# zheminzhou/PEPPAN

Hardware: AMD Instinct MI355X
Metric: gene_pairs_aligned_per_s (higher is better)
Workload: dtype int16; 1 GPU; synthgenes-v1 seed 355: 10000 genes x 1002 nt, all-vs-all (BASELINE configs[2] search stage), min_id 0.45 min_ratio...; queries_per_rank=10000, reference_genes_per_rank=10000

## Files before the change

peppan_amd/csrc/capi.hip:

```cpp
#include "common.h"
#include "setstate.h"
#include <chrono>
#include <time.h>
#include <algorithm>
#include <cmath>
#include <cstring>
#include <new>

int pep_fail(pep_ctx *ctx, int code, const std::string &msg)
{
    if (ctx) { ctx->n_down = 0; ctx->pin_down_used = 0; }
    if (ctx) {
        ctx->err = msg;
        ctx->n_pending = 0;
        ctx->pin_small_used = 0;
        for (LookbackState &st : ctx->lookback) st.dirty = true;
        ctx->zero_clean = false;
        for (bool &f : ctx->zero_ok) f = false;
        ctx->set_clean_slots = 0;
    }
    return code;
}

int dev_reserve(pep_ctx *ctx, DevBuf &b, size_t bytes)
// ... 459 lines not shown
int32_t pep_min_score_ka(uint32_t qlen, double dbsize, double max_evalue, double ka_lambda, double ka_k)
{
    const double s = log(ka_k * (double)qlen * dbsize / max_evalue) / ka_lambda;
    const int32_t r = (int32_t)ceil(s);
    return r < 1 ? 1 : r;
}

int32_t pep_min_score(uint32_t qlen, double dbsize, double max_evalue)
{
    return pep_min_score_ka(qlen, dbsize, max_evalue, 0.267, 0.041);
}

int pep_ctx_create(int device, pep_ctx **out)
{
    if (!out) return PEP_ERR_ARG;
    *out = nullptr;
    int n = 0;
    if (hipGetDeviceCount(&n) != hipSuccess || device < 0 || device >= n) return PEP_ERR_HIP;
    pep_ctx *ctx = new (std::nothrow) pep_ctx();
    if (!ctx) return PEP_ERR_INTERNAL;
    ctx->device = device;
    memset(&ctx->stats, 0, sizeof(ctx->stats));
    pep_default_params(&ctx->params);
    if (hipSetDevice(device) != hipSuccess) { delete ctx; return PEP_ERR_HIP; }
    if (hipStreamCreate(&ctx->stream.s) != hipSuccess) { delete ctx; return PEP_ERR_HIP; }
    if (pin_reserve(ctx, ctx->pin_small, 16384) != PEP_OK) { *out = ctx; return PEP_ERR_HIP; }
    int rc = pep_selftest_dpp(ctx);
    if (rc != PEP_OK) { *out = ctx; return rc; }
    *out = ctx;
    return PEP_OK;
}

pep_ctx::~pep_ctx()
{
    (void)hipSetDevice(device);
    pep_drop_dev_result(this);
    pep_materialise_staged(this);
}

void pep_ctx_destroy(pep_ctx *ctx) { delete ctx; }

int pep_live_resources(uint64_t *device_bytes, uint64_t *pinned_bytes, uint32_t *events)
{
    if (!device_bytes || !pinned_bytes || !events) return PEP_ERR_ARG;
    *device_bytes = pep_live.device_bytes; *pinned_bytes = pep_live.pinned_bytes; *events = pep_live.events;
    return PEP_OK;
// ... 456 lines not shown
```

peppan_amd/csrc/common.h:

```cpp
#pragma once
#include <hip/hip_runtime.h>
#include <stdint.h>
#include <stddef.h>
#include <atomic>
#include <optional>
#include <string>
#include <type_traits>
#include <vector>
#include "../../include/peppan_hip.h"
using CallTimes = struct pep_call_times;

#define PEP_WAVE 64
#define PEP_TAB_REP 16

#define PEP_HIP(ctx, expr)                                                                            \
    do {                                                                                              \
        hipError_t _e = (expr);                                                                       \
        if (_e != hipSuccess) {                                                                       \
            return pep_fail((ctx), PEP_ERR_HIP, std::string(#expr) + ": " + hipGetErrorString(_e));   \
        }                                                                                             \
    } while (0)

#define PEP_TRY(expr)                  \
    do {                               \
        int _rc = (expr);              \
        if (_rc != PEP_OK) return _rc; \
// ... 121 lines not shown
    PEP_WS_TRACE_DIRS = PEP_WS_IDX_PART,
    PEP_WS_SW_SCAN_IN = 14,
    PEP_WS_SW_ORDER = 15,
    PEP_WS_SEL = 19,
    PEP_WS_SEL_RUNS_KEYS = 20,
    PEP_WS_RUNS = 21,
    PEP_WS_KEEP = 22,
    PEP_WS_HITS_OUT = 23,
    PEP_WS_COUNT
};

enum PepLookback {
    PEP_LB_SCAN_U32 = 0,
    PEP_LB_SCAN_U64,
    PEP_LB_SELECT_COUNT,
    PEP_LB_SELECT_RUNS,
    PEP_LB_TOPK_HITS,
    PEP_LB_TOPK_RUNS,
    PEP_LB_SORT,
    PEP_LB_COUNT
};

struct LookbackState { DevBuf buf; uint32_t epoch = 0, ticket_base = 0; bool dirty = false; };

enum PepTimer { TM_SEED = 0, TM_TOTAL, TM_SW, TM_SW_TRACE, TM_TRACE, TM_MATCH0, TM_MATCH1, TM_MATCH2, TM_MATCH3, TM_COUNT };

struct pep_ctx {
    int device = 0;
    Stream stream;
    PinBuf pin_small;
    size_t pin_small_used = 0;
    struct PendingRead { void *dst; size_t off, n; } pending[32];
    int n_pending = 0;
    PinBuf pin_k1, pin_k1q;
    DevBuf d_k1_desc_q, d_k1_desc_t;
    DevBuf d_self_delta, d_self_t;
    const uint32_t *self_first = nullptr;
    uint32_t self_first_cnt = 0;
    int self_exact_len = 0;
    Event k1_event;
    Event k1q_event;
    Event wait_event;
    Event k1_t0, k1_t1;
    PinBuf pin_up;
    size_t pin_up_used = 0;
    Event up_event;
// ... 30 lines not shown
        std::vector<pep_target_meta> t_meta;
        DevBuf d_off, d_len, d_desc;
        DevBuf d_first;
        uint32_t n_first = 0;
    } nucl_q, nucl_t;
    int nucl_strands = 0;
    DevBuf d_min_score;
    DevBuf d_trace_defer;
    DevBuf d_trace_mode;
    std::vector<uint32_t> group_of_seq;
    DevBuf d_t_class;
    DevBuf d_t_subject;
    DevBuf ws[PEP_WS_COUNT];
    DevBuf sub_lds;
    DevBuf d_params;
    int8_t d_params_host[1024] = {};
    bool d_params_valid = false;
    Event tm_a[TM_COUNT], tm_b[TM_COUNT];
    int tm_state[TM_COUNT] = {};
    int timing_level = 0;
    PinBuf pin_labels;
    uint64_t trace_swept = 0;
    LookbackState lookback[PEP_LB_COUNT];
    DevBuf sort_hist;
    DevBuf d_set;
    uint64_t set_clean_slots = 0;
    DevBuf uf_nodes;
    std::vector<uint32_t> uf_nodes_host;
    struct { bool pending = false; pep_result *res = nullptr; const void *d_hits = nullptr, *d_cig = nullptr; const uint32_t *d_n_hits = nullptr; uint64_t n_bound = 0; bool grouped = false; } ext;
    struct { void *d_dst = nullptr; const void *pinned_src = nullptr; uint64_t n_words = 0; } upload;
    bool want_nt_match = false;
    DevBuf d_nt_match;
    PinBuf pin_nt_match;
    uint32_t grp_nodes = 0, grp_q_base = 0;
    bool device_results = false;
    pep_result *dev_result = nullptr;
    DevBuf d_zero;
    bool zero_clean = false;
    DevBuf d_mail_copy;
    bool zero_ok[4] = {false, false, false, false};
    CallTimes calls[PEP_CALL_COUNT] = {};
    uint64_t k16_serial = 0;
    DevBuf k16_tri, k16_leader;
    DevBuf k17[11];
    uint64_t k18_n_conf = 0, k18_n_walk = 0;
    DevBuf k18[18];
// ... 102 lines not shown
int pep_read_back_with_upload(pep_ctx *ctx, void *dst, const void *d_src, size_t n, void *d_up_dst, const void *pinned_up_src, uint64_t n_up_words);
struct pep_key_unpack { int on, tb, bb; uint32_t bin_min; };
int pep_sort_u64(pep_ctx *ctx, uint64_t *d_keys, uint64_t *d_tmp, const uint32_t *d_n, uint64_t n_bound, int bits, uint32_t *d_hist_zeroed,
                 const pep_key_unpack *unpack);
int pep_sort_u64_two_level(pep_ctx *ctx, uint64_t *d_keys, uint64_t *d_tmp, uint64_t n, int bits, const uint32_t *d_top_hist, const pep_key_unpack *unpack);
int pep_k1_query_queue(pep_ctx *ctx, int gtable), pep_k1_query_take(pep_ctx *ctx);
int pep_k1_ref_queue(pep_ctx *ctx, int frames, int gtable), pep_k1_ref_take(pep_ctx *ctx);
int pep_k1_host_tables(pep_ctx *ctx, PepSide side);
int pep_nucl_sets(pep_ctx *ctx, int strands);
int pep_find_candidates(pep_ctx *ctx, uint64_t **d_cands, uint64_t *n_cands, int (*before_sync)(pep_ctx *) = nullptr, int (*need_targets)(pep_ctx *) = nullptr);
int pep_upload_sub_table(pep_ctx *ctx);
int pep_sw_run(pep_ctx *ctx, const uint64_t *d_cands, uint64_t n, bool trace, const int32_t *d_known = nullptr, const int32_t *d_end_lane = nullptr, const int32_t *d_skip_mode = nullptr,
               const uint32_t *d_n = nullptr, uint64_t dir_blocks_bound = 0, unsigned long long **d_hdr = nullptr);
int pep_extend(pep_ctx *ctx, const uint64_t *d_cands, uint64_t n_cands, const int32_t *h_min_score, pep_result *res, bool defer = false, bool group = false);
int pep_extend_finish(pep_ctx *ctx);
int pep_selftest_dpp(pep_ctx *ctx);
int pep_k7_hits_queue(pep_ctx *ctx, uint64_t n_hits, const pep_hit *d_hits, const uint32_t *d_cigar, const uint32_t *d_n_hits = nullptr);
int pep_k10_queue(pep_ctx *ctx, uint64_t n_hits, const pep_hit *d_hits, const uint32_t *d_n_hits = nullptr);
int pep_k10_components_dev(pep_ctx *ctx, uint32_t n_nodes, uint64_t n_hits, const pep_hit *d_hits, uint32_t q_base, const uint32_t *h_node_of_target,
                           uint64_t n_targets, uint32_t *h_label);

static inline uint64_t ceil_div(uint64_t a, uint64_t b) { return (a + b - 1) / b; }

__device__ __forceinline__ unsigned long long pep_band_cells(int Lq, int Lt, int dlo)
{
    const int dl = max(dlo, -(Lq - 1)), dh = min(dlo + 127, Lt - 1);
    if (dl > dh) return 0ull;
    auto tri = [](long long a, long long b) { return b < a ? 0ll : (a + b) * (b - a + 1) / 2; };
    const long long k = (long long)Lt - Lq;
    const long long flat_hi = min((long long)dh, k), slope_lo = max((long long)dl, k + 1);
    long long total = (flat_hi >= dl ? (flat_hi - dl + 1) * (long long)Lq : 0ll);
    if (slope_lo <= dh) total += (long long)(dh - slope_lo + 1) * Lt - tri(slope_lo, dh);
    total += tri(dl, min((long long)dh, -1ll));
    return (unsigned long long)total;
}

__device__ __forceinline__ uint32_t uf_root(uint32_t *parent, uint32_t x)
{
    for (;;) {
        const uint32_t p = __hip_atomic_load(&parent[x], __ATOMIC_RELAXED, __HIP_MEMORY_SCOPE_AGENT);
        if (p == x) return x;
        x = p;
    }
}
__device__ __forceinline__ void uf_unite(uint32_t *parent, uint32_t x, uint32_t y)
{
// ... 15 lines not shown
```

peppan_amd/csrc/sw.hip:

```cpp
#include "common.h"
#include "lookback.h"

namespace {

constexpr int LDS_TABLE_BYTES = 256 * PEP_TAB_REP * 4;
constexpr int TAB_ROW_SHIFT = PEP_TAB_REP == 32 ? 7 : 6;
constexpr int WAVES_PER_BLOCK = 8;

constexpr int LEN_BUCKETS = 1024;
__device__ __forceinline__ uint32_t len_bucket(uint32_t nb) { return nb < (uint32_t)LEN_BUCKETS ? nb : (uint32_t)LEN_BUCKETS - 1; }

struct SwArgs {
    const uint64_t *cands;
    uint64_t n;
    const uint8_t *q_res, *t_res;
    const uint32_t *q_off, *q_len, *t_off, *t_len;
    const uint32_t *sub_image;
    const uint64_t *dir_off;
    const uint32_t *nblk;
    uint32_t *dirs;
    int4 *out;
    int oe, ext;
    int lds_res_bytes;
    uint32_t *defer;
// ... 578 lines not shown
}

__global__ __launch_bounds__(64 * WAVES_PER_BLOCK, 4) void sw_trace_retry_kernel(SwArgs a)
{
    extern __shared__ __attribute__((aligned(16))) unsigned char smem[];
    const unsigned long long n_list = a.counts[6];
    if ((unsigned long long)blockIdx.x * WAVES_PER_BLOCK >= n_list) return;
    uint32_t *lds_tab = reinterpret_cast<uint32_t *>(smem);
    for (int x = threadIdx.x; x < LDS_TABLE_BYTES / 4; x += blockDim.x) lds_tab[x] = a.sub_image[x];
    __syncthreads();
    const int lane = threadIdx.x & 63, wave = threadIdx.x >> 6;
    uint16_t *lds_res = reinterpret_cast<uint16_t *>(smem + LDS_TABLE_BYTES + (size_t)wave * a.lds_res_bytes);
    const SwArgs *ka = (const SwArgs *)__builtin_amdgcn_kernarg_segment_ptr();
    for (;;) {
        unsigned long long w = 0;
        if (lane == 0) w = atomicAdd(a.counts + 7, 1ull);
        w = ((unsigned long long)(unsigned int)__builtin_amdgcn_readfirstlane((int)(w >> 32)) << 32) | (unsigned int)__builtin_amdgcn_readfirstlane((int)w);
        if (w >= n_list) break;
        trace_slow_path(ka, (uint64_t)a.defer[w], smem, lds_res, lane, 1);
    }
}

struct IdentArgs { int8_t diag[32]; uint32_t dominant, harmless; };
__global__ __launch_bounds__(256) void identical_check(const uint64_t *__restrict__ cands, uint64_t n, const uint8_t *__restrict__ q_res, const uint32_t *__restrict__ q_off,
                                                       const uint32_t *__restrict__ q_len, const uint8_t *__restrict__ t_res, const uint32_t *__restrict__ t_off,
                                                       const uint32_t *__restrict__ t_len, IdentArgs ia, int4 *__restrict__ out, int32_t *__restrict__ settled)
{
    const int lane = threadIdx.x & 63;
    const uint64_t c = (uint64_t)blockIdx.x * 4 + (threadIdx.x >> 6);
    if (c >= n) return;
    const uint64_t key = cands[c];
    const uint32_t q = (uint32_t)(key >> 43), t = (uint32_t)((key >> 18) & ((1u << 25) - 1));
    const int bin = (int)(key & ((1u << 18) - 1));
    const int dlo = bin * 64 - (1 << 23) - 32;
    const int L = (int)q_len[q];
    const int my_diag = ia.diag[lane & 31];
    bool same = L > 0 && L == (int)t_len[t] && dlo <= 0 && dlo + 127 >= 0;
    bool tail = false;
    int sum = 0;
    if (same) {
        const uint8_t *qg = q_res + q_off[q], *tg = t_res + t_off[t];
        for (int x0 = 0; x0 < L && same; x0 += 256) {
            uint32_t qa[4], ta[4];
#pragma unroll
            for (int k = 0; k < 4; ++k) { const int x = x0 + 64 * k + lane; qa[k] = x < L ? qg[x] : 0u; ta[k] = x < L ? tg[x] : 0u; }
#pragma unroll
            for (int k = 0; k < 4; ++k) {
                const bool in = x0 + 64 * k + lane < L;
                const int d = __shfl(my_diag, (int)(qa[k] & 31u), 64);
                const bool dom = in && qa[k] < 32u && ((ia.dominant >> qa[k]) & 1u), harm = in && qa[k] < 32u && ((ia.harmless >> qa[k]) & 1u);
                const unsigned long long m_dom = __ballot(dom), m_harm = __ballot(harm);
                const bool bad = __ballot(in && (qa[k] != ta[k] || !(dom || harm))) != 0ull
                                 || (m_dom && (tail || (m_harm && (63 - __builtin_clzll(m_dom)) > (__builtin_ffsll((long long)m_harm) - 1))));
                if (bad) same = false;
                if (dom) sum += d;
                tail = tail || m_harm != 0ull;
            }
        }
    }
#pragma unroll
    for (int d = 32; d > 0; d >>= 1) sum += __shfl_xor(sum, d, 64);
    same = same && sum > 0;
    if (lane == 0) {
        settled[c] = same ? -2 : 0;
        if (same) out[c] = make_int4(sum, (-dlo) >> 1, -1, (-dlo) >> 1);
    }
}

__global__ __launch_bounds__(256) void sw_prep(const uint64_t *__restrict__ cands, uint64_t n_host, const uint32_t *__restrict__ d_n, const uint32_t *__restrict__ q_len,
                                               const uint32_t *__restrict__ t_len, uint32_t *__restrict__ nblk, uint64_t *__restrict__ nblk64,
                                               unsigned long long *__restrict__ cells_total,
                                               uint32_t *__restrict__ len_hist,
                                               uint32_t nb_limit,
                                               const int32_t *__restrict__ skip_mode,
                                               int count_skipped,
                                               uint64_t *__restrict__ dir_off,
                                               LbLaunch lb)
{
    __shared__ uint32_t lh[LEN_BUCKETS];
    __shared__ uint32_t s_tile;
    for (int x = threadIdx.x; x < LEN_BUCKETS; x += 256) lh[x] = 0;
    __syncthreads();
    const uint64_t n = d_n ? (uint64_t)*d_n : n_host;
    const uint32_t tile = lb.state ? lb_take_tile(lb.state, lb.ticket_base, &s_tile) : blockIdx.x;
    const uint64_t c = (uint64_t)tile * 256 + threadIdx.x;
    unsigned long long cells = 0, blocks = 0, cells_skipped = 0, n_skipped = 0;
    bool is_long = false;
    const bool skipped = c < n && skip_mode && skip_mode[c] == -2;
// ... 139 lines not shown
    PEP_TRY(pep_zero_block(ctx, trace ? PEP_ZC_SW_TRACE : PEP_ZC_SW_SCORE, trace ? PEP_ZERO_SW_TRACE : PEP_ZERO_SW_SCORE, PEP_ZERO_SW_BYTES, &zb));
    PEP_TRY(dev_reserve(ctx, ctx->ws[PEP_WS_SW_ORDER], (n + 1) * sizeof(uint32_t)));
    unsigned long long *cells = reinterpret_cast<unsigned long long *>(zb);
    if (d_hdr) *d_hdr = cells;
    uint32_t *len_hist = reinterpret_cast<uint32_t *>(reinterpret_cast<unsigned char *>(zb) + 64), *cursor = len_hist + LEN_BUCKETS, *order = ctx->ws[PEP_WS_SW_ORDER].as<uint32_t>();
    LbLaunch lb = {nullptr, 0, 0};
    const uint64_t prep_tiles = ceil_div(n + (trace ? 1 : 0), 256);
    if (trace) PEP_TRY(pep_lookback_begin(ctx, PEP_LB_SCAN_U64, prep_tiles, 1, 48, &lb));
    const int32_t *skip = trace ? d_skip_mode : nullptr;
    if (!trace && (P.reserved2 & 2) == 0 && (n >= 16384 || (P.reserved2 & 4)) && P.gap_ext >= 0 && P.gap_open + P.gap_ext > 0) {
        PEP_TRY(dev_reserve(ctx, ctx->ws[PEP_WS_SW_SKIP_MODE], (n + 1) * sizeof(int32_t)));
        IdentArgs ia;
        ia.dominant = ia.harmless = 0;
        for (int r = 0; r < 32; ++r) {
            ia.diag[r] = P.sub[r * 32 + r];
            bool dom = P.sub[r * 32 + r] > 0, harm = true;
            for (int x = 0; x < 32; ++x) {
                if (x != r) dom = dom && P.sub[r * 32 + x] < P.sub[r * 32 + r];
                harm = harm && P.sub[r * 32 + x] <= 0;
            }
            if (dom) ia.dominant |= 1u << r;
            if (harm) ia.harmless |= 1u << r;
        }
        hipLaunchKernelGGL(identical_check, dim3((unsigned)ceil_div(n, 4)), dim3(256), 0, ctx->stream, d_cands, n, ctx->q.res.as<const uint8_t>(), ctx->q.off.as<const uint32_t>(),
                           ctx->q.len.as<const uint32_t>(), ctx->t.res.as<const uint8_t>(), ctx->t.off.as<const uint32_t>(), ctx->t.len.as<const uint32_t>(), ia,
                           ctx->ws[PEP_WS_SW_OUT].as<int4>(), ctx->ws[PEP_WS_SW_SKIP_MODE].as<int32_t>());
        skip = ctx->ws[PEP_WS_SW_SKIP_MODE].as<const int32_t>();
    }
    hipLaunchKernelGGL(sw_prep, dim3((unsigned)prep_tiles), dim3(256), 0, ctx->stream, d_cands, n, trace ? d_n : nullptr, ctx->q.len.as<const uint32_t>(),
                       ctx->t.len.as<const uint32_t>(), ctx->ws[PEP_WS_SW_NBLK].as<uint32_t>(), ctx->ws[PEP_WS_SW_SCAN_IN].as<uint64_t>(), cells, len_hist, nb_limit, skip, trace ? 0 : 1,
                       ctx->ws[PEP_WS_SW_DIR_OFF].as<uint64_t>(), lb);
    hipLaunchKernelGGL(sw_order, dim3((unsigned)ceil_div(n, 256)), dim3(256), 0, ctx->stream, ctx->ws[PEP_WS_SW_NBLK].as<const uint32_t>(), n, trace ? d_n : nullptr,
                       (const uint32_t *)len_hist, cursor, order, skip);
    if (trace) {
        uint64_t total_blk = dir_blocks_bound;
        if (!dir_blocks_bound) {
            unsigned long long h_tot[6] = {0, 0, 0, 0, 0, 0};
            PEP_TRY(pep_read_back(ctx, h_tot, cells, sizeof(h_tot)));
            PEP_TRY(pep_sync_reads(ctx));
            total_blk = h_tot[1];
            ctx->trace_swept = h_tot[5];
            ctx->stats.cells_trace += h_tot[0];
            ctx->stats.cells_swept_trace += total_blk * 16 * 64;
            ctx->stats.dir_bytes += total_blk * 512;
        }
        PEP_TRY(dev_reserve(ctx, ctx->ws[PEP_WS_TRACE_DIRS], total_blk * 512 + 512));
        PEP_TRY(dev_reserve(ctx, ctx->d_trace_mode, (n + 1) * sizeof(int32_t)));
// ... 48 lines not shown
```

peppan_amd/csrc/translate.hip:

```cpp
#include "common.h"
#include "lookback.h"
#include "setstate.h"
#include <algorithm>

namespace {

__constant__ uint8_t c_codon[2][64];

__device__ __forceinline__ int base2(uint8_t ch)
{
    const uint32_t u = ch & 0xDFu;
    const int code = (int)(((u >> 1) ^ (u >> 2)) & 3u);
    if (u == ((0x54474341u >> (code * 8)) & 0xFFu)) return code;
    return ch == '-' ? -2 : -1;
}

__device__ __forceinline__ void nt4(uint32_t w, bool rev, uint32_t &pk, uint32_t &bad)
{
    const uint32_t u = w & 0xDFDFDFDFu;
    uint32_t code = ((u >> 1) ^ (u >> 2)) & 0x03030303u;
    const uint32_t diff = u ^ __builtin_amdgcn_perm(0u, 0x54474341u, code);
    const uint32_t nz = ((((diff & 0x7F7F7F7Fu) + 0x7F7F7F7Fu) | diff) >> 7) & 0x01010101u;
    if (rev) code ^= 0x03030303u;
    pk = (code * 0x40100401u) >> 24;
// ... 20 lines not shown
    return c_codon[tab][(b[0] << 4) | (b[1] << 2) | b[2]];
}

__device__ __forceinline__ int64_t frame_len(int64_t L, int frame)
{
    const int64_t rem = L - (frame <= 3 ? frame - 1 : frame - 4);
    return rem > 0 ? (rem + 2) / 3 : 0;
}

struct K1Summary {
    unsigned long long residues, total;
    uint32_t n, max_len;
    uint32_t pad[2];
};
static_assert(sizeof(K1Summary) == 2 * 16, "the summary takes two descriptor slots");


struct K1Src { uint64_t off; uint32_t L, pad; };
static_assert(sizeof(K1Src) == sizeof(PackDesc), "source records lie behind the descriptors, in slots of the same size");
__host__ __device__ __forceinline__ K1Src *k1_src_of(const PackDesc *desc, uint32_t cap) { return reinterpret_cast<K1Src *>(const_cast<PackDesc *>(desc) + cap + 3); }

__device__ __forceinline__ uint32_t padded_len(uint32_t len) { return (len + 15u) / 16u * 16u + PEP_SEQ_GAP; }

__global__ __launch_bounds__(256) void k1_query_frames(const uint8_t *__restrict__ nt, const uint64_t *__restrict__ off, uint32_t n, int tab,
                                                       PackDesc *__restrict__ desc, uint32_t *__restrict__ padded, uint32_t *__restrict__ len_out, uint32_t *__restrict__ n_out,
                                                       K1Summary *__restrict__ sum, uint32_t *__restrict__ pin_len, K1Src *__restrict__ src_of)
{
    const int lane = threadIdx.x & 63;
    const uint32_t g = blockIdx.x * 4 + (threadIdx.x >> 6);
    if (blockIdx.x == 0 && threadIdx.x == 0) { *n_out = n; sum->residues = 0ull; sum->max_len = 0u; }
    if (g >= n) return;
    const uint64_t o = off[g];
    const uint8_t *s = nt + o;
    const int L = (int)(off[g + 1] - o);
    __shared__ uint32_t stage_all[4][392];
    uint32_t *stage = stage_all[threadIdx.x >> 6];
    const unsigned long long stop_codon = __ballot(c_codon[tab][lane] == 23);
    const int na1 = (int)frame_len(L, 1), na2 = (int)frame_len(L, 2), na3 = (int)frame_len(L, 3);
    uint32_t x1 = 0, x2 = 0, x3 = 0;
    for (int c0 = 0; c0 + 1 < na1; c0 += 512) {
        const int lo = 3 * c0;
        const uintptr_t A = reinterpret_cast<uintptr_t>(s + lo);
        const int shift = (int)(A & 3u);
        const uint32_t *al = reinterpret_cast<const uint32_t *>(A - shift);
        const int n_dw = (min(1538, L - lo) + shift + 3) >> 2;
        for (int x = lane; x < n_dw; x += 64) stage[x] = al[x];
        __builtin_amdgcn_fence(__ATOMIC_RELEASE, "workgroup");
        __builtin_amdgcn_wave_barrier();
        __builtin_amdgcn_fence(__ATOMIC_ACQUIRE, "workgroup");
        uint32_t raw[8];
#pragma unroll
        for (int k = 0; k < 8; ++k) raw[k] = stage[6 * lane + k];
        unsigned long long codes = 0;
        uint32_t bad = 0, gap = 0;
#pragma unroll
        for (int k = 0; k < 7; ++k) {
            const uint32_t w = __builtin_amdgcn_alignbyte(raw[k + 1], raw[k], (uint32_t)shift);
            uint32_t pk, bd;
            nt4(w, false, pk, bd);
            const uint32_t g = w ^ 0x2D2D2D2Du;
// ... 11 lines not shown
        for (int h = 0; h < 8; ++h) {
            const int a = c0 + 8 * lane + h;
#pragma unroll
            for (int f = 0; f < 3; ++f) {
                const int j = 3 * h + f;
                const uint32_t idx = (uint32_t)(codes >> (50 - 2 * j)) & 63u;
                const uint32_t b3 = (bad >> (25 - j)) & 7u, g3 = (gap >> (25 - j)) & 7u;
                const bool stop = g3 == 0u && (b3 != 0u || ((stop_codon >> idx) & 1ull));
                *cnt[f] += (a + 1 < lim[f] && stop) ? 1u : 0u;
            }
        }
        __builtin_amdgcn_wave_barrier();
    }
    for (int d = 32; d > 0; d >>= 1) { x1 += __shfl_xor(x1, d, 64); x2 += __shfl_xor(x2, d, 64); x3 += __shfl_xor(x3, d, 64); }
    uint32_t best_cnt = x1, best_f = 1, best_len = (uint32_t)na1;
    if (x2 < best_cnt) { best_cnt = x2; best_f = 2; best_len = (uint32_t)na2; }
    if (x3 < best_cnt) { best_cnt = x3; best_f = 3; best_len = (uint32_t)na3; }
    if (lane == 0) {
        desc[g] = PackDesc{g, best_f, 0u, best_len};
        src_of[g] = K1Src{o, (uint32_t)L, 0u};
        padded[g] = padded_len(best_len);
        len_out[g] = best_len;
        pin_len[g] = best_len;
    }
}

__device__ __forceinline__ int64_t chunk_end(const uint8_t *s, int64_t L, int f, int tab, int64_t na, int64_t c0, int lane)
{
    if (na + 1 - c0 < 1001) return na;
    int64_t x0 = c0 + 1000;
    for (;;) {
        const int64_t a = x0 + lane;
        bool isx = false;
        if (a < na) { bool gap; isx = (translate_at(s, (int)L, f, (int)a, tab, &gap) == 23) && !gap; }
        else if (a == na) isx = true;
        const unsigned long long m = __ballot(isx);
        if (m) return x0 + (int64_t)__ffsll((long long)m) - 1;
        x0 += 64;
    }
}

constexpr int64_t K1_LONG = 98304;
struct K1Seg { uint32_t w, seg; };
constexpr uint32_t K1_FILL_FROM = 128;
static_assert((int64_t)K1_FILL_FROM * 1001 > K1_LONG, "a frame that leaves its descriptors to k1_ref_desc_fill is a long one");
struct K1Long { uint32_t w, pad; uint64_t mask_off; };
// ... 130 lines not shown
    if (w >= (uint64_t)n * n_frames) return;
    const uint32_t g = (uint32_t)(w / n_frames);
    const int f = (int)(w % n_frames) + 1;
    const uint8_t *s = nt + off[g];
    const int64_t L = (int64_t)(off[g + 1] - off[g]);
    const int64_t na = frame_len(L, f);
    if (na + 1 > long_from) return;
    const uint64_t base = chunk_base[w];
    uint32_t cnt = 0;
    int64_t c0 = 0;
    while (c0 < na + 1) {
        const int64_t end = chunk_end(s, L, f, tab, na, c0, lane);
        int64_t len = end - c0 + 1;
        if (end == na) --len;
        if (len > 0) {
            if (lane == 0) { chunk_off[base + cnt] = (uint32_t)c0; chunk_len[base + cnt] = (uint32_t)len; }
            ++cnt;
        }
        c0 = end + 1;
    }
    if (lane == 0) chunk_cnt[w] = cnt;
}

__global__ __launch_bounds__(256) void k1_pack(const uint8_t *__restrict__ nt, const K1Src *__restrict__ src_of, int tab,
                                               const PackDesc *__restrict__ desc, const uint32_t *__restrict__ pk_off, const uint32_t *__restrict__ n_ptr, uint32_t cap,
                                               uint8_t *__restrict__ res, uint2 *__restrict__ blk2seq, const K1Summary *__restrict__ d_sum, K1Summary *__restrict__ pin_sum)
{
    const int lane = threadIdx.x & 63;
    const uint32_t s = blockIdx.x * 4 + (threadIdx.x >> 6);
    if (blockIdx.x == 0 && threadIdx.x == 0) *pin_sum = *d_sum;
    const uint32_t n_packed = *n_ptr;
    const uint32_t sc = min(s, cap);
    const PackDesc d = desc[sc];
    const K1Src so = src_of[sc];
    const uint32_t start = pk_off[sc], next = pk_off[sc + 1];
    __shared__ uint32_t codon_all[4][64];
    uint32_t *codon = codon_all[threadIdx.x >> 6];
    codon[lane] = c_codon[tab][lane];
    if (n_packed == 0) {
        if (s == 0) for (uint32_t x = lane; x < pk_off[0]; x += 64) res[x] = (uint8_t)PEP_PAD_CODE;
        return;
    }
    if (s >= n_packed) return;
    const uint8_t *src = nt + so.off;
    const int L = (int)so.L;
    if (s == 0) for (uint32_t x = lane; x < start; x += 64) res[x] = (uint8_t)PEP_PAD_CODE;
    __shared__ uint32_t stage_all[4][392];
    uint32_t *stage = stage_all[threadIdx.x >> 6];
    const int frame = (int)d.frame;
    const bool fwd = frame <= 3;
    const int fo = fwd ? frame - 1 : frame - 4;
    for (uint32_t c0 = 0; c0 < next - start; c0 += 512) {
        const int P0 = fo + 3 * (int)(d.aa_off + c0);
        const int lo = fwd ? P0 : L - 1 - (P0 + 1535);
        int shift = 0;
        if (c0 < d.len && P0 < L) {
            const uintptr_t A = reinterpret_cast<uintptr_t>(src) + (intptr_t)lo;
            shift = (int)(A & 3u);
            const uint32_t *al = reinterpret_cast<const uint32_t *>(A - shift);
            const int first_dw = lo < 0 ? (-lo + shift) >> 2 : 0;
            const int n_dw = (min(1536, L - lo) + shift + 3) >> 2;
            for (int x = first_dw + lane; x < n_dw; x += 64) stage[x] = al[x];
        }
        __builtin_amdgcn_fence(__ATOMIC_RELEASE, "workgroup");
        __builtin_amdgcn_wave_barrier();
        __builtin_amdgcn_fence(__ATOMIC_ACQUIRE, "workgroup");
        const uint32_t x0 = c0 + 8 * lane;
        if (x0 < next - start) {
            const int di = fwd ? 6 * lane : 378 - 6 * lane;
            uint32_t raw[7], ch[6];
#pragma unroll
// ... 14 lines not shown
            for (int h = 0; h < 2; ++h) {
                uint32_t pk[3], bad[3];
#pragma unroll
                for (int k = 0; k < 3; ++k) nt4(ch[3 * h + k], !fwd, pk[k], bad[k]);
                const uint32_t codes = (pk[0] << 16) | (pk[1] << 8) | pk[2];
                uint32_t bad12 = (bad[0] << 8) | (bad[1] << 4) | bad[2];
                const int nv = min(max(n_valid - 12 * h, 0), 12);
                bad12 |= (1u << (12 - nv)) - 1u;
                uint32_t w = 0;
#pragma unroll
                for (int k = 0; k < 4; ++k) {
                    uint32_t c = codon[(codes >> (18 - 6 * k)) & 63u];
                    if ((bad12 >> (9 - 3 * k)) & 7u) c = 23u;
                    if (4 * h + k >= n_res) c = PEP_PAD_CODE;
                    w |= c << (8 * k);
                }
                word[h] = w;
            }
            *reinterpret_cast<uint2 *>(res + start + x0) = make_uint2(word[0], word[1]);
        }
        __builtin_amdgcn_wave_barrier();
    }
    for (uint32_t b = (start >> 5) + lane, last = ((next & 31u) == 16u) ? ((next - 16u) >> 5) - 1u : (next - 17u) >> 5; b <= last && last != ~0u; b += 64) blk2seq[b] = make_uint2(s, start);
}

constexpr uint32_t NUCL_SLICE = 32768;
__global__ __launch_bounds__(256) void nucl_pack(const uint8_t *__restrict__ nt, const uint64_t *__restrict__ nt_off, const NuclDesc *__restrict__ desc,
                                                 const uint32_t *__restrict__ pk_off, uint32_t n_packed, uint8_t *__restrict__ res, uint2 *__restrict__ blk2seq)
{
    const int lane = threadIdx.x & 63;
    const uint32_t s = blockIdx.x * 4 + (threadIdx.x >> 6);
    if (n_packed == 0) {
        if (s == 0) for (uint32_t x = lane; x < pk_off[0]; x += 64) res[x] = (uint8_t)PEP_PAD_CODE;
        return;
    }
    if (s >= n_packed) return;
    const NuclDesc d = desc[s];
    const uint32_t start = pk_off[s], next = pk_off[s + 1];
    const uint8_t *src = nt + nt_off[d.seq];
    const int64_t L = (int64_t)(nt_off[d.seq + 1] - nt_off[d.seq]);
    const uint32_t x_lo = blockIdx.y * NUCL_SLICE, x_hi = min(next - start, x_lo + NUCL_SLICE);
    if (x_lo >= next - start) return;
    if (s == 0 && blockIdx.y == 0) for (uint32_t x = lane; x < start; x += 64) res[x] = (uint8_t)PEP_PAD_CODE;
    for (uint32_t x0 = x_lo + 8 * lane; x0 < x_hi; x0 += 512) {
        uint32_t word[2] = {0, 0};
        uint8_t raw[8];
// ... 129 lines not shown
        if (bm) { atomicAdd(&sum->residues, blk_s[0] + blk_s[1] + blk_s[2] + blk_s[3]); atomicMax(&sum->max_len, bm); }
    }
    if (i == cap) { sum->n = n; sum->total = (unsigned long long)at + 2ull * PEP_END_PAD; }
}

int reserve_packed(pep_ctx *ctx, SeqSet &out, uint32_t cap, uint64_t upper)
{
    if (upper > PEP_MAX_RESIDUES + (uint64_t)cap * 32) return pep_fail(ctx, PEP_ERR_LIMIT, "packed protein set exceeds 2^29 bytes");
    PEP_TRY(dev_reserve(ctx, out.res, upper + 64));
    PEP_TRY(dev_reserve(ctx, out.off, ((size_t)cap + 2) * 4));
    PEP_TRY(dev_reserve(ctx, out.len, ((size_t)cap + 2) * 4));
    PEP_TRY(dev_reserve(ctx, out.blk2seq, (upper / 32 + 2) * sizeof(uint2)));
    return PEP_OK;
}

int layout_and_pack(pep_ctx *ctx, const NtSet &nt, int tab, const PackDesc *d_desc, const uint32_t *d_padded, uint32_t cap, const uint32_t *d_n,
                    SeqSet &out, K1Summary *pin_sum)
{
    K1Summary *d_sum = reinterpret_cast<K1Summary *>(const_cast<PackDesc *>(d_desc) + cap);
    LbLaunch sc;
    const uint64_t tiles = ceil_div((uint64_t)cap + 1, 256);
    PEP_TRY(pep_lookback_begin(ctx, PEP_LB_SCAN_U32, tiles, 1, 32, &sc));
    hipLaunchKernelGGL(k1_offsets, dim3((unsigned)tiles), dim3(256), 0, ctx->stream, d_n, d_padded, cap, out.off.as<uint32_t>(), out.len.as<const uint32_t>(), d_sum, sc);
    hipLaunchKernelGGL(k1_pack, dim3((unsigned)ceil_div((uint64_t)cap + 1, 4)), dim3(256), 0, ctx->stream, nt.nt.as<const uint8_t>(), (const K1Src *)k1_src_of(d_desc, cap), tab,
                       d_desc, out.off.as<const uint32_t>(), d_n, cap, out.res.as<uint8_t>(), out.blk2seq.as<uint2>(), (const K1Summary *)d_sum, pin_sum);
    PEP_HIP(ctx, hipGetLastError());
    return PEP_OK;
}

int k1_take(pep_ctx *ctx, hipEvent_t ev, const void *pinned, SeqSet &out)
{
    PEP_HIP(ctx, pep_event_wait(ev));
    const K1Summary *sum = reinterpret_cast<const K1Summary *>(pinned);
    if (sum->total > PEP_MAX_RESIDUES) return pep_fail(ctx, PEP_ERR_LIMIT, "packed protein set exceeds 2^29 bytes");
    if (sum->max_len > PEP_MAX_SEQ_LEN) return pep_fail(ctx, PEP_ERR_LIMIT, "protein longer than PEP_MAX_SEQ_LEN");
    out.n = sum->n; out.total = sum->total; out.residues = sum->residues; out.max_len = sum->max_len;
    return PEP_OK;
}

enum {
    K1Q_PADDED = 3,
    K1Q_COUNT = 5,
    K1R_CHUNK_CNT = 1, K1R_CHUNK_OFF, K1R_CHUNK_LEN,
    K1R_FIRST = 5,
    K1R_PADDED,
    K1_SLOTS
};
static_assert(K1Q_COUNT < K1_SLOTS && K1_SLOTS <= PEP_WS_HITS_OUT, "leaves the device-resident hit table alone");

}

int pep_k1_query_queue(pep_ctx *ctx, int gtable)
{
    const NtSet &nt = ctx->q_nt;
    const int tab = gtable == 4 ? 1 : 0;
    const uint32_t n = nt.n;
    PEP_TRY(upload_codon_table(ctx));
    DevBuf *W = ctx->ws;
    DevBuf &D = ctx->d_k1_desc_q;
    PEP_TRY(dev_reserve(ctx, D, (2 * (size_t)n + 4) * sizeof(PackDesc)));
    PEP_TRY(pin_reserve(ctx, ctx->pin_k1q, sizeof(K1Summary) + ((size_t)n + 1) * 4));
    K1Summary *pin_sum = reinterpret_cast<K1Summary *>(ctx->pin_k1q.p);
    uint32_t *pin_len = reinterpret_cast<uint32_t *>(ctx->pin_k1q.p + sizeof(K1Summary));
    PEP_TRY(dev_reserve(ctx, W[K1Q_PADDED], ((size_t)n + 1) * 4));
    PEP_TRY(dev_reserve(ctx, W[K1Q_COUNT], 16));
    const uint64_t upper = 2 * PEP_END_PAD + (nt.total + 2 * (uint64_t)n) / 3 + (uint64_t)n * (16 + PEP_SEQ_GAP);
    PEP_TRY(reserve_packed(ctx, ctx->q, n, upper));
    if (n) hipLaunchKernelGGL(k1_query_frames, dim3((unsigned)ceil_div(n, 4)), dim3(256), 0, ctx->stream, nt.nt.as<const uint8_t>(), nt.off.as<const uint64_t>(), n, tab,
                              D.as<PackDesc>(), W[K1Q_PADDED].as<uint32_t>(), ctx->q.len.as<uint32_t>(), W[K1Q_COUNT].as<uint32_t>(), reinterpret_cast<K1Summary *>(D.as<PackDesc>() + n), pin_len,
                              k1_src_of(D.as<const PackDesc>(), n));
    else hipLaunchKernelGGL(k1_query_desc, dim3(1), dim3(64), 0, ctx->stream, 0u, (const uint32_t *)nullptr, (const uint32_t *)nullptr,
                            D.as<PackDesc>(), W[K1Q_PADDED].as<uint32_t>(), ctx->q.len.as<uint32_t>(), W[K1Q_COUNT].as<uint32_t>(), reinterpret_cast<K1Summary *>(D.as<PackDesc>() + n), pin_len);
    PEP_TRY(layout_and_pack(ctx, nt, tab, D.as<const PackDesc>(), W[K1Q_PADDED].as<const uint32_t>(), n, W[K1Q_COUNT].as<const uint32_t>(), ctx->q, pin_sum));
    if (!ctx->k1q_event.ensure(pep_wait_event_flags())) return pep_fail(ctx, PEP_ERR_HIP, "hipEventCreate failed");
    PEP_HIP(ctx, hipEventRecord(ctx->k1q_event, ctx->stream));
    return PEP_OK;
}

int pep_k1_query_take(pep_ctx *ctx)
{
    PEP_TRY(k1_take(ctx, ctx->k1q_event, ctx->pin_k1q.p, ctx->q));
    const uint32_t *pin_len = reinterpret_cast<const uint32_t *>(ctx->pin_k1q.p + sizeof(K1Summary));
    ctx->q.h_len.assign(pin_len, pin_len + ctx->q_nt.n);
    return PEP_OK;
}

int pep_k1_host_tables(pep_ctx *ctx, PepSide side)
{
    if (ctx->side[side].tables_built) return PEP_OK;
    SeqSet &set = pep_set_of(ctx, side);
    const DevBuf &D = side == PEP_SIDE_Q ? ctx->d_k1_desc_q : ctx->d_k1_desc_t;
// ... 237 lines not shown
```

Before: 25.85 million gene-pairs/s.

## Convert per-wave item kernels to persistent grid-stride loops with header prefetch

Three kernels (query frame translation, packing, identical-pair check) now launch only as many blocks as can be resident, sized from an occupancy query, and each wave walks items with a grid stride instead of one wave per item. Each iteration prefetches the next item's header (offsets, lengths, descriptors) to hide global load latency, and shared-memory setup and the codon table load are amortised across items. This cuts block launch and scheduling overhead but may lose load balance when item costs vary. An environment variable can cap the grid size.

```diff
diff --git a/peppan_amd/csrc/capi.hip b/peppan_amd/csrc/capi.hip
--- a/peppan_amd/csrc/capi.hip
+++ b/peppan_amd/csrc/capi.hip
@@ -505,6 +505,7 @@
     ctx->device = device;
     memset(&ctx->stats, 0, sizeof(ctx->stats));
     pep_default_params(&ctx->params);
+    if (const char *e = getenv("PEPPAN_HIP_ITEM_BLOCKS")) ctx->item_blocks_cap = (unsigned)std::min<long>(std::max<long>(atol(e), 0L), 1L << 20);
     if (hipSetDevice(device) != hipSuccess) { delete ctx; return PEP_ERR_HIP; }
     if (hipStreamCreate(&ctx->stream.s) != hipSuccess) { delete ctx; return PEP_ERR_HIP; }
     if (pin_reserve(ctx, ctx->pin_small, 16384) != PEP_OK) { *out = ctx; return PEP_ERR_HIP; }
diff --git a/peppan_amd/csrc/common.h b/peppan_amd/csrc/common.h
--- a/peppan_amd/csrc/common.h
+++ b/peppan_amd/csrc/common.h
@@ -2,6 +2,7 @@
 #include <hip/hip_runtime.h>
 #include <stdint.h>
 #include <stddef.h>
+#include <algorithm>
 #include <atomic>
 #include <optional>
 #include <string>
@@ -169,6 +170,8 @@
 };
 
 struct LookbackState { DevBuf buf; uint32_t epoch = 0, ticket_base = 0; bool dirty = false; };
+
+enum PepItemKernel { PEP_ITEM_QUERY_FRAMES = 0, PEP_ITEM_PACK, PEP_ITEM_IDENTICAL, PEP_ITEM_COUNT };
 
 enum PepTimer { TM_SEED = 0, TM_TOTAL, TM_SW, TM_SW_TRACE, TM_TRACE, TM_MATCH0, TM_MATCH1, TM_MATCH2, TM_MATCH3, TM_COUNT };
 
@@ -245,6 +248,8 @@
     PinBuf pin_labels;
     uint64_t trace_swept = 0;
     LookbackState lookback[PEP_LB_COUNT];
+    unsigned item_resident[PEP_ITEM_COUNT] = {};
+    unsigned item_blocks_cap = 0;
     DevBuf sort_hist;
     DevBuf d_set;
     uint64_t set_clean_slots = 0;
@@ -393,6 +398,32 @@
 
 static inline uint64_t ceil_div(uint64_t a, uint64_t b) { return (a + b - 1) / b; }
 
+struct ItemLoop {
+    uint64_t i, stride, n;
+    __device__ __forceinline__ explicit ItemLoop(uint64_t n_items)
+        : i((uint64_t)__builtin_amdgcn_readfirstlane((int)(blockIdx.x * 4u + (threadIdx.x >> 6)))), stride((uint64_t)gridDim.x * 4u), n(n_items) {}
+    __device__ __forceinline__ bool live() const { return i < n; }
+    __device__ __forceinline__ void next() { i += stride; }
+    __device__ __forceinline__ uint64_t at(int k) const { return at(k, n - 1); }
+    __device__ __forceinline__ uint64_t at(int k, uint64_t last) const { const uint64_t x = i + (uint64_t)k * stride; return x < last ? x : last; }
+};
+
+template <class Kernel>
+int pep_item_grid(pep_ctx *ctx, PepItemKernel which, Kernel kernel, uint64_t n_items, unsigned *grid)
+{
+    if (!ctx->item_resident[which]) {
+        int per_cu = 0, n_cu = 0;
+        PEP_HIP(ctx, hipOccupancyMaxActiveBlocksPerMultiprocessor(&per_cu, kernel, 256, 0));
+        PEP_HIP(ctx, hipDeviceGetAttribute(&n_cu, hipDeviceAttributeMultiprocessorCount, ctx->device));
+        if (per_cu < 1 || n_cu < 1) return pep_fail(ctx, PEP_ERR_INTERNAL, "pep_item_grid: no resident block");
+        ctx->item_resident[which] = (unsigned)per_cu * (unsigned)n_cu;
+    }
+    uint64_t g = std::min<uint64_t>(std::max<uint64_t>(ceil_div(n_items, 4), 1), ctx->item_resident[which]);
+    if (ctx->item_blocks_cap) g = std::min<uint64_t>(g, ctx->item_blocks_cap);
+    *grid = (unsigned)g;
+    return PEP_OK;
+}
+
 __device__ __forceinline__ unsigned long long pep_band_cells(int Lq, int Lt, int dlo)
 {
     const int dl = max(dlo, -(Lq - 1)), dh = min(dlo + 127, Lt - 1);
diff --git a/peppan_amd/csrc/sw.hip b/peppan_amd/csrc/sw.hip
--- a/peppan_amd/csrc/sw.hip
+++ b/peppan_amd/csrc/sw.hip
@@ -624,24 +624,27 @@
 }
 
 struct IdentArgs { int8_t diag[32]; uint32_t dominant, harmless; };
-__global__ __launch_bounds__(256) void identical_check(const uint64_t *__restrict__ cands, uint64_t n, const uint8_t *__restrict__ q_res, const uint32_t *__restrict__ q_off,
-                                                       const uint32_t *__restrict__ q_len, const uint8_t *__restrict__ t_res, const uint32_t *__restrict__ t_off,
-                                                       const uint32_t *__restrict__ t_len, IdentArgs ia, int4 *__restrict__ out, int32_t *__restrict__ settled)
-{
-    const int lane = threadIdx.x & 63;
-    const uint64_t c = (uint64_t)blockIdx.x * 4 + (threadIdx.x >> 6);
-    if (c >= n) return;
-    const uint64_t key = cands[c];
-    const uint32_t q = (uint32_t)(key >> 43), t = (uint32_t)((key >> 18) & ((1u << 25) - 1));
-    const int bin = (int)(key & ((1u << 18) - 1));
-    const int dlo = bin * 64 - (1 << 23) - 32;
-    const int L = (int)q_len[q];
+struct IdentHead { uint32_t q, t; int dlo, Lq, Lt; uint32_t qo, to; };
+__device__ __forceinline__ IdentHead ident_head(uint64_t key, const uint32_t *__restrict__ q_off, const uint32_t *__restrict__ q_len, const uint32_t *__restrict__ t_off,
+                                                const uint32_t *__restrict__ t_len)
+{
+    IdentHead h;
+    h.q = (uint32_t)(key >> 43); h.t = (uint32_t)((key >> 18) & ((1u << 25) - 1));
+    h.dlo = (int)(key & ((1u << 18) - 1)) * 64 - (1 << 23) - 32;
+    h.Lq = (int)q_len[h.q]; h.Lt = (int)t_len[h.t]; h.qo = q_off[h.q]; h.to = t_off[h.t];
+    return h;
+}
+
+__device__ __forceinline__ void identical_item(uint64_t c, const IdentHead &h, int lane, const uint8_t *__restrict__ q_res, const uint8_t *__restrict__ t_res, const IdentArgs &ia,
+                                               int4 *__restrict__ out, int32_t *__restrict__ settled)
+{
+    const int dlo = h.dlo, L = h.Lq;
     const int my_diag = ia.diag[lane & 31];
-    bool same = L > 0 && L == (int)t_len[t] && dlo <= 0 && dlo + 127 >= 0;
+    bool same = L > 0 && L == h.Lt && dlo <= 0 && dlo + 127 >= 0;
     bool tail = false;
     int sum = 0;
     if (same) {
-        const uint8_t *qg = q_res + q_off[q], *tg = t_res + t_off[t];
+        const uint8_t *qg = q_res + h.qo, *tg = t_res + h.to;
         for (int x0 = 0; x0 < L && same; x0 += 256) {
             uint32_t qa[4], ta[4];
 #pragma unroll
@@ -666,6 +669,22 @@
     if (lane == 0) {
         settled[c] = same ? -2 : 0;
         if (same) out[c] = make_int4(sum, (-dlo) >> 1, -1, (-dlo) >> 1);
+    }
+}
+
+__global__ __launch_bounds__(256) void identical_check(const uint64_t *__restrict__ cands, uint64_t n, const uint8_t *__restrict__ q_res, const uint32_t *__restrict__ q_off,
+                                                       const uint32_t *__restrict__ q_len, const uint8_t *__restrict__ t_res, const uint32_t *__restrict__ t_off,
+                                                       const uint32_t *__restrict__ t_len, IdentArgs ia, int4 *__restrict__ out, int32_t *__restrict__ settled)
+{
+    const int lane = threadIdx.x & 63;
+    ItemLoop it(n);
+    if (!it.live()) return;
+    IdentHead cur = ident_head(cands[it.at(0)], q_off, q_len, t_off, t_len), nxt;
+    uint64_t key_ahead = cands[it.at(1)];
+    for (; it.live(); it.next(), cur = nxt) {
+        nxt = ident_head(key_ahead, q_off, q_len, t_off, t_len);
+        key_ahead = cands[it.at(2)];
+        identical_item(it.i, cur, lane, q_res, t_res, ia, out, settled);
     }
 }
 
@@ -851,7 +870,9 @@
             if (dom) ia.dominant |= 1u << r;
             if (harm) ia.harmless |= 1u << r;
         }
-        hipLaunchKernelGGL(identical_check, dim3((unsigned)ceil_div(n, 4)), dim3(256), 0, ctx->stream, d_cands, n, ctx->q.res.as<const uint8_t>(), ctx->q.off.as<const uint32_t>(),
+        unsigned ident_grid = 0;
+        PEP_TRY(pep_item_grid(ctx, PEP_ITEM_IDENTICAL, identical_check, n, &ident_grid));
+        hipLaunchKernelGGL(identical_check, dim3(ident_grid), dim3(256), 0, ctx->stream, d_cands, n, ctx->q.res.as<const uint8_t>(), ctx->q.off.as<const uint32_t>(),
                            ctx->q.len.as<const uint32_t>(), ctx->t.res.as<const uint8_t>(), ctx->t.off.as<const uint32_t>(), ctx->t.len.as<const uint32_t>(), ia,
                            ctx->ws[PEP_WS_SW_OUT].as<int4>(), ctx->ws[PEP_WS_SW_SKIP_MODE].as<int32_t>());
         skip = ctx->ws[PEP_WS_SW_SKIP_MODE].as<const int32_t>();
diff --git a/peppan_amd/csrc/translate.hip b/peppan_amd/csrc/translate.hip
--- a/peppan_amd/csrc/translate.hip
+++ b/peppan_amd/csrc/translate.hip
@@ -66,20 +66,16 @@
 
 __device__ __forceinline__ uint32_t padded_len(uint32_t len) { return (len + 15u) / 16u * 16u + PEP_SEQ_GAP; }
 
-__global__ __launch_bounds__(256) void k1_query_frames(const uint8_t *__restrict__ nt, const uint64_t *__restrict__ off, uint32_t n, int tab,
-                                                       PackDesc *__restrict__ desc, uint32_t *__restrict__ padded, uint32_t *__restrict__ len_out, uint32_t *__restrict__ n_out,
-                                                       K1Summary *__restrict__ sum, uint32_t *__restrict__ pin_len, K1Src *__restrict__ src_of)
-{
-    const int lane = threadIdx.x & 63;
-    const uint32_t g = blockIdx.x * 4 + (threadIdx.x >> 6);
-    if (blockIdx.x == 0 && threadIdx.x == 0) { *n_out = n; sum->residues = 0ull; sum->max_len = 0u; }
-    if (g >= n) return;
-    const uint64_t o = off[g];
+struct K1Head { uint64_t o, end; };
+__device__ __forceinline__ K1Head k1_head(const uint64_t *__restrict__ off, uint64_t g) { return K1Head{off[g], off[g + 1]}; }
+
+__device__ __forceinline__ void k1_query_item(uint32_t g, const K1Head &h, int lane, uint32_t *stage, unsigned long long stop_codon, const uint8_t *__restrict__ nt,
+                                              PackDesc *__restrict__ desc, uint32_t *__restrict__ padded, uint32_t *__restrict__ len_out, uint32_t *__restrict__ pin_len,
+                                              K1Src *__restrict__ src_of)
+{
+    const uint64_t o = h.o;
     const uint8_t *s = nt + o;
-    const int L = (int)(off[g + 1] - o);
-    __shared__ uint32_t stage_all[4][392];
-    uint32_t *stage = stage_all[threadIdx.x >> 6];
-    const unsigned long long stop_codon = __ballot(c_codon[tab][lane] == 23);
+    const int L = (int)(h.end - o);
     const int na1 = (int)frame_len(L, 1), na2 = (int)frame_len(L, 2), na3 = (int)frame_len(L, 3);
     uint32_t x1 = 0, x2 = 0, x3 = 0;
     for (int c0 = 0; c0 + 1 < na1; c0 += 512) {
@@ -137,6 +133,24 @@
         padded[g] = padded_len(best_len);
         len_out[g] = best_len;
         pin_len[g] = best_len;
+    }
+}
+
+__global__ __launch_bounds__(256) void k1_query_frames(const uint8_t *__restrict__ nt, const uint64_t *__restrict__ off, uint32_t n, int tab,
+                                                       PackDesc *__restrict__ desc, uint32_t *__restrict__ padded, uint32_t *__restrict__ len_out, uint32_t *__restrict__ n_out,
+                                                       K1Summary *__restrict__ sum, uint32_t *__restrict__ pin_len, K1Src *__restrict__ src_of)
+{
+    const int lane = threadIdx.x & 63;
+    if (blockIdx.x == 0 && threadIdx.x == 0) { *n_out = n; sum->residues = 0ull; sum->max_len = 0u; }
+    __shared__ uint32_t stage_all[4][392];
+    uint32_t *stage = stage_all[threadIdx.x >> 6];
+    const unsigned long long stop_codon = __ballot(c_codon[tab][lane] == 23);
+    ItemLoop it(n);
+    if (!it.live()) return;
+    K1Head cur = k1_head(off, it.at(0)), nxt;
+    for (; it.live(); it.next(), cur = nxt) {
+        nxt = k1_head(off, it.at(1));
+        k1_query_item((uint32_t)it.i, cur, lane, stage, stop_codon, nt, desc, padded, len_out, pin_len, src_of);
     }
 }
 
@@ -313,31 +327,21 @@
     if (lane == 0) chunk_cnt[w] = cnt;
 }
 
-__global__ __launch_bounds__(256) void k1_pack(const uint8_t *__restrict__ nt, const K1Src *__restrict__ src_of, int tab,
-                                               const PackDesc *__restrict__ desc, const uint32_t *__restrict__ pk_off, const uint32_t *__restrict__ n_ptr, uint32_t cap,
-                                               uint8_t *__restrict__ res, uint2 *__restrict__ blk2seq, const K1Summary *__restrict__ d_sum, K1Summary *__restrict__ pin_sum)
-{
-    const int lane = threadIdx.x & 63;
-    const uint32_t s = blockIdx.x * 4 + (threadIdx.x >> 6);
-    if (blockIdx.x == 0 && threadIdx.x == 0) *pin_sum = *d_sum;
-    const uint32_t n_packed = *n_ptr;
-    const uint32_t sc = min(s, cap);
-    const PackDesc d = desc[sc];
-    const K1Src so = src_of[sc];
-    const uint32_t start = pk_off[sc], next = pk_off[sc + 1];
-    __shared__ uint32_t codon_all[4][64];
-    uint32_t *codon = codon_all[threadIdx.x >> 6];
-    codon[lane] = c_codon[tab][lane];
-    if (n_packed == 0) {
-        if (s == 0) for (uint32_t x = lane; x < pk_off[0]; x += 64) res[x] = (uint8_t)PEP_PAD_CODE;
-        return;
-    }
-    if (s >= n_packed) return;
+struct PackHead { PackDesc d; K1Src so; uint32_t start, next; };
+__device__ __forceinline__ PackHead pack_head(uint64_t s, const PackDesc *__restrict__ desc, const K1Src *__restrict__ src_of, const uint32_t *__restrict__ pk_off)
+{
+    return PackHead{desc[s], src_of[s], pk_off[s], pk_off[s + 1]};
+}
+
+__device__ __forceinline__ void k1_pack_item(uint32_t s, const PackHead &h, int lane, const uint32_t *codon, uint32_t *stage, const uint8_t *__restrict__ nt,
+                                             uint8_t *__restrict__ res, uint2 *__restrict__ blk2seq)
+{
+    const PackDesc d = h.d;
+    const K1Src so = h.so;
+    const uint32_t start = h.start, next = h.next;
     const uint8_t *src = nt + so.off;
     const int L = (int)so.L;
     if (s == 0) for (uint32_t x = lane; x < start; x += 64) res[x] = (uint8_t)PEP_PAD_CODE;
-    __shared__ uint32_t stage_all[4][392];
-    uint32_t *stage = stage_all[threadIdx.x >> 6];
     const int frame = (int)d.frame;
     const bool fwd = frame <= 3;
     const int fo = fwd ? frame - 1 : frame - 4;
@@ -398,6 +402,28 @@
         __builtin_amdgcn_wave_barrier();
     }
     for (uint32_t b = (start >> 5) + lane, last = ((next & 31u) == 16u) ? ((next - 16u) >> 5) - 1u : (next - 17u) >> 5; b <= last && last != ~0u; b += 64) blk2seq[b] = make_uint2(s, start);
+}
+
+__global__ __launch_bounds__(256) void k1_pack(const uint8_t *__restrict__ nt, const K1Src *__restrict__ src_of, int tab,
+                                               const PackDesc *__restrict__ desc, const uint32_t *__restrict__ pk_off, const uint32_t *__restrict__ n_ptr, uint32_t cap,
+                                               uint8_t *__restrict__ res, uint2 *__restrict__ blk2seq, const K1Summary *__restrict__ d_sum, K1Summary *__restrict__ pin_sum)
+{
+    const int lane = threadIdx.x & 63;
+    if (blockIdx.x == 0 && threadIdx.x == 0) *pin_sum = *d_sum;
+    __shared__ uint32_t codon_all[4][64];
+    __shared__ uint32_t stage_all[4][392];
+    uint32_t *codon = codon_all[threadIdx.x >> 6], *stage = stage_all[threadIdx.x >> 6];
+    codon[lane] = c_codon[tab][lane];
+    ItemLoop it(*n_ptr);
+    PackHead cur = pack_head(it.at(0, cap), desc, src_of, pk_off), nxt;
+    if (it.n == 0) {
+        if (it.i == 0) for (uint32_t x = lane; x < cur.start; x += 64) res[x] = (uint8_t)PEP_PAD_CODE;
+        return;
+    }
+    for (; it.live(); it.next(), cur = nxt) {
+        nxt = pack_head(it.at(1, cap), desc, src_of, pk_off);
+        k1_pack_item((uint32_t)it.i, cur, lane, codon, stage, nt, res, blk2seq);
+    }
 }
 
 constexpr uint32_t NUCL_SLICE = 32768;
@@ -573,7 +599,9 @@
     const uint64_t tiles = ceil_div((uint64_t)cap + 1, 256);
     PEP_TRY(pep_lookback_begin(ctx, PEP_LB_SCAN_U32, tiles, 1, 32, &sc));
     hipLaunchKernelGGL(k1_offsets, dim3((unsigned)tiles), dim3(256), 0, ctx->stream, d_n, d_padded, cap, out.off.as<uint32_t>(), out.len.as<const uint32_t>(), d_sum, sc);
-    hipLaunchKernelGGL(k1_pack, dim3((unsigned)ceil_div((uint64_t)cap + 1, 4)), dim3(256), 0, ctx->stream, nt.nt.as<const uint8_t>(), (const K1Src *)k1_src_of(d_desc, cap), tab,
+    unsigned pack_grid = 0;
+    PEP_TRY(pep_item_grid(ctx, PEP_ITEM_PACK, k1_pack, (uint64_t)cap + 1, &pack_grid));
+    hipLaunchKernelGGL(k1_pack, dim3(pack_grid), dim3(256), 0, ctx->stream, nt.nt.as<const uint8_t>(), (const K1Src *)k1_src_of(d_desc, cap), tab,
                        d_desc, out.off.as<const uint32_t>(), d_n, cap, out.res.as<uint8_t>(), out.blk2seq.as<uint2>(), (const K1Summary *)d_sum, pin_sum);
     PEP_HIP(ctx, hipGetLastError());
     return PEP_OK;
@@ -617,7 +645,9 @@
     PEP_TRY(dev_reserve(ctx, W[K1Q_COUNT], 16));
     const uint64_t upper = 2 * PEP_END_PAD + (nt.total + 2 * (uint64_t)n) / 3 + (uint64_t)n * (16 + PEP_SEQ_GAP);
     PEP_TRY(reserve_packed(ctx, ctx->q, n, upper));
-    if (n) hipLaunchKernelGGL(k1_query_frames, dim3((unsigned)ceil_div(n, 4)), dim3(256), 0, ctx->stream, nt.nt.as<const uint8_t>(), nt.off.as<const uint64_t>(), n, tab,
+    unsigned frames_grid = 0;
+    if (n) PEP_TRY(pep_item_grid(ctx, PEP_ITEM_QUERY_FRAMES, k1_query_frames, n, &frames_grid));
+    if (n) hipLaunchKernelGGL(k1_query_frames, dim3(frames_grid), dim3(256), 0, ctx->stream, nt.nt.as<const uint8_t>(), nt.off.as<const uint64_t>(), n, tab,
                               D.as<PackDesc>(), W[K1Q_PADDED].as<uint32_t>(), ctx->q.len.as<uint32_t>(), W[K1Q_COUNT].as<uint32_t>(), reinterpret_cast<K1Summary *>(D.as<PackDesc>() + n), pin_len,
                               k1_src_of(D.as<const PackDesc>(), n));
     else hipLaunchKernelGGL(k1_query_desc, dim3(1), dim3(64), 0, ctx->stream, 0u, (const uint32_t *)nullptr, (const uint32_t *)nullptr,
```

Measured after the change: 25.96 million gene-pairs/s (median of 2 runs). About the same (+0.4%).
